# thenumbernine/lua-multigrid-poisson

Hardware: AMD Instinct MI355X
Metric: V-cycles/sec + finest-smoother achieved HBM GB/s, 3D Poisson (higher is better)
Workload: dtype f32; 1 GPU; BASELINE configs[2]: 3D Poisson 512^3 per GPU, 7-point, RB-GS 2+2, V-cycle, trilinear P, 2x2x2-average R, consistent coarse boundary, per-cycle RMS-update err; parallelism=single GPU, levels=10

## Files before the change

### lua-multigrid-poisson_amd/csrc/mgp_internal.h

```cpp
#pragma once
#include <hip/hip_runtime.h>
#include <cstdint>

namespace mgp {

constexpr int kGhost3D = 1;
constexpr int kGhostZs = 5;
constexpr int kZsHaloPre = 5, kZsHaloPost = 4, kZsHaloCoarse = 3;

struct Geo {
    int nx, ny;
    int lx, ly;
    int hw, lhw;
    int64_t nz;
    int64_t H;
    int64_t P;
    int64_t z0;
    int64_t gnz;
};

constexpr int kRealF32D = 12;

hipError_t launch_init_point_charge(int rb, int dim, void* u, void* f, Geo g, int64_t cx, int64_t cy,
                                    int64_t cz, hipStream_t s);
// ... 8 lines not shown

int half_blocks(int rb, Geo g, bool gs);
hipError_t launch_half_sweep(int rb, int dim, bool fine, int color, const void* other, const void* f, void* dst,
                             const void* old, double* partials, Geo g, double h, double cl, bool gs, hipStream_t s);
bool fresh_supported(int rb, const Geo& g);
hipError_t launch_fresh_sweep(int rb, int dim, const void* f, void* u, Geo g, double h, double cl, hipStream_t s,
                              bool store_red = true);
bool post1_supported(int rb, const Geo& g, const Geo& gc);
hipError_t launch_post_first(int rb, int dim, int linear, void* u, const void* V, const void* f, Geo g, Geo gc,
                             double h, double cl, double clc, hipStream_t s);
hipError_t launch_residual_restrict(int rb, int dim, const void* u, const void* f, void* R, Geo g, Geo gc, double h,
                                    double cl, hipStream_t s);
bool bres_supported(int rb, const Geo& g);
hipError_t launch_black_residual_restrict(int rb, int dim, void* u, const void* f, void* R, Geo g, Geo gc, double h,
                                          double cl, hipStream_t s);
hipError_t launch_rb_sweep(int rb, int dim, const void* src, const void* f, void* dst, Geo g, double h, double cl,
                           bool store_red, hipStream_t s);
hipError_t launch_residual_field_v(int rb, int dim, const void* u, const void* f, void* r, Geo g, double h, double cl,
                                   hipStream_t s);
hipError_t launch_fw_restrict(int rb, int dim, const void* r, void* R, Geo g, Geo gc, double clc, hipStream_t s);
bool resfw_supported(int rb, int dim, const Geo& g, int gz, bool dist);
hipError_t launch_resfw(int rb, int dim, const void* u, const void* f, void* R, Geo g, Geo gc, double h, double cl,
                        double clc, int gz, hipStream_t s);
hipError_t launch_prolong_correct(int rb, int dim, int linear, void* u, const void* V, Geo g, Geo gc, double clc,
                                  hipStream_t s, bool black_only = false);
hipError_t launch_sqdiff_sum(int rb, const void* a, const void* b, int64_t n, double* partials, double* out,
                             hipStream_t s, int* ctr = nullptr);
hipError_t launch_nonfinite_check(int rb, const void* p, int64_t n, int id, int* first, hipStream_t s);
hipError_t launch_metrics(int rb, const void* psi, const void* old, int64_t n, double* partials, double* out,
                          hipStream_t s);
int resnorm_blocks(int rb, Geo g);
hipError_t launch_residual_norm(int rb, int dim, const void* u, const void* f, Geo g, double h, double cl,
                                double* partials, double* out, hipStream_t s);
int sum_scratch(int n);
hipError_t launch_sum_partials(const double* partials, int n, double* out, hipStream_t s, int* ctr = nullptr);

int defect_blocks(Geo g);
int refine_add_blocks(Geo g);
int refine_partials();
hipError_t launch_defect(int dim, const double* psi64, const double* f64, float* r32, float* u32_or_null, Geo g,
                         double h, double* partials, double* out, hipStream_t s);
hipError_t launch_refine_add(double* psi64, const float* e32, Geo g, double* partials, double* out, hipStream_t s);
hipError_t launch_refine_widen(const float* src, double* dst, int64_t n, hipStream_t s);
hipError_t launch_refine_narrow(const double* src, float* dst, int64_t n, hipStream_t s);

struct FusedTuning {
    bool wide = true;
    int ys_half = -1;
    int ys_rows = 32;
    int64_t wgs = 256;
    int patch_pre = 0, patch_post = -1;
    bool fwf = true;
    int post_zc = 256;
    bool stamp_r = false;
};
FusedTuning fused_tuning_from_env();

struct LaunchInfo {
    char name[96];
    int64_t grid;
};

struct FusedArgs {
    FusedTuning tu;
    LaunchInfo* info;
    bool pre;
    int linear;
    const void* src;
    const void* f;
    void* dst;
    const void* old;
    void* R;
    const void* V;
    double* partials;
    Geo g, gc;
    double h, cl, clc;
    int zc;
    int ghost;
};
bool fused_supported(int rb, int dim, int ns, const Geo& g, const FusedTuning& tu);
hipError_t prepare_kernels(int rb);
int fused_zc(int rb, const Geo& g, bool pre, bool clz, const FusedTuning& tu);
int fused_blocks(int rb, const Geo& g, int zc, bool clz, const FusedTuning& tu);
hipError_t launch_fused(int rb, const FusedArgs& a, hipStream_t s);
bool fused_fwf_supported(int rb, int dim, bool clz, bool dist, const FusedTuning& tu);

constexpr int kBlkMaxSweeps = 2;
constexpr int kBlkTile = 8;
constexpr int kBlkTile2D = 32;
struct BlockArgs {
    bool pre;
    int linear;
    int ns;
    const void* src;
    const void* f;
    void* dst;
    void* R;
    const void* V;
    Geo g, gc;
    double h, cl, clc;
};
bool block_supported(int rb, int dim, int ns, const Geo& g);
hipError_t launch_block(int rb, int dim, const BlockArgs& a, hipStream_t s);

struct Block2Args {
    bool pre;
// ... 62 lines not shown
```

### lua-multigrid-poisson_amd/csrc/mgp_kernels.hip

```cpp
#include "mgp_device.h"

#include <cstdio>
#include <cstdlib>
#include <type_traits>
#include <utility>

namespace mgp {
namespace {




constexpr unsigned kMaxBlocks = 1u << 20;
inline unsigned nblk_gs(int64_t n)
{
    const int64_t b = (n + kBlock - 1) / kBlock;
    return (unsigned)(b < (int64_t)kMaxBlocks ? (b > 0 ? b : 1) : kMaxBlocks);
}

template <typename T>
__global__ __launch_bounds__(kBlock) void k_init(T* __restrict__ u, T* __restrict__ f, Geo g, int64_t cx, int64_t cy,
                                                 int64_t cz, int dim3)
{
    const int64_t n = g.P * g.nz;
// ... 1636 lines not shown
        const bool ox = (o == 0 && I0 + e == 0) || (o == 1 && I0 + e == cx - 1);
        auto col = [&](const T (&cc)[N + 2]) { return ox ? cc[pe] : (o ? cc[e + 2] : cc[e]); };
        const T a0 = w0 * c0[pe] + w1 * sv(col(c0), ox, false);
        const T a1 = w0 * sv(c1[pe], false, oy) + w1 * sv(col(c1), ox, oy);
        b[e] = w0 * a0 + w1 * a1;
    }
}

template <int NTL>
__device__ __forceinline__ void block_partial_t(double acc, double* partials)
{
    __shared__ double red[NTL];
    red[threadIdx.x] = acc;
    __syncthreads();
    for (int w = 512; w > 0; w >>= 1) {
        if ((int)threadIdx.x < w && (int)threadIdx.x + w < NTL) red[threadIdx.x] += red[threadIdx.x + w];
        __syncthreads();
    }
    if (threadIdx.x == 0) partials[blockIdx.x] = red[0];
}

#ifndef ZS_WPE_PRE
#define ZS_WPE_PRE 2
#endif
#ifndef ZS_PFD_PRE
#define ZS_PFD_PRE 2
#endif
#ifndef ZS_PFD_POST
#define ZS_PFD_POST 1
#endif
#ifndef ZS_PFD_PRE_CL
#define ZS_PFD_PRE_CL 1
#endif
template <typename F, int... K>
__device__ __forceinline__ void zs_unroll_impl(F& f, std::integer_sequence<int, K...>)
{
    (f(std::integral_constant<int, K>()), ...);
}
template <int U, typename F>
__device__ __forceinline__ void zs_unroll(F&& f)
{
    zs_unroll_impl(f, std::make_integer_sequence<int, U>());
}
#ifndef ZS_BQ
#define ZS_BQ 1
#endif
#ifndef ZS_RASK
#define ZS_RASK 1
#endif
constexpr bool kZsRask = ZS_RASK != 0;
#ifndef ZS_WPE_POST
#define ZS_WPE_POST 4
#endif
template <typename T, bool PRE, int LINEAR, bool ERR, bool CLZ, bool WIDE = false>
__global__ __launch_bounds__((ZsShape<T, PRE, CLZ, WIDE, PRE && LINEAR == 2>::NTL))
__attribute__((amdgpu_waves_per_eu(1, PRE ? ZS_WPE_PRE : ZS_WPE_POST))) void k_zs(const T* __restrict__ src, const T* __restrict__ f,
                                                                T* __restrict__ dst, const T* old, T* __restrict__ R,
                                                                const T* __restrict__ V, double* __restrict__ partials,
                                                                Geo g, Geo gc, Op<T, 3> op, T clc, int zc, int gz,
                                                                int patch)
{
    constexpr bool FWF = PRE && LINEAR == 2;
    using S = ZsShape<T, PRE, CLZ, WIDE, FWF>;
    constexpr int N = S::N, H = S::H, HWE = S::HWE, G = S::G, YE = S::YE, SLOT = S::SLOT, TX = S::TX,
                  TY = S::TY, NS3 = S::NS3, NTL = S::NTL;
    constexpr bool RR = PRE && LINEAR == 0;
    constexpr bool ZSRC = PRE && ERR;
    using VT = Vec<T, N>;
    using PF = ZsPrefetch<T, N>;
    constexpr int PFD = PRE ? (CLZ ? ZS_PFD_PRE : ZS_PFD_PRE_CL) : ZS_PFD_POST, NPF = PFD + 1, UNR = NPF == 3 ? 12 : 4;
    static_assert(PFD >= 1 && PFD <= 3, "prefetch distance 1..3");
    extern __shared__ __align__(16) unsigned char zs_smem[];
    T* const lds = reinterpret_cast<T*>(zs_smem);
    const int tid = threadIdx.x;

    const int tiles_x = g.nx / TX, tiles_y = g.ny / TY;
    const int b = xcd_remap(blockIdx.x, gridDim.x);
    const int tile = b % (tiles_x * tiles_y);
    const int Z0 = (b / (tiles_x * tiles_y)) * zc;
    int tx_ = tile % tiles_x, ty_ = tile / tiles_x;
    if (patch) {
        const int px = patch & 255, py = patch >> 8, per = px * py, prow = tiles_x / px;
        const int pi = tile / per, q = tile % per;
        tx_ = (pi % prow) * px + q % px;
        ty_ = (pi / prow) * py + q / px;
    }
    const int X0 = tx_ * TX, Y0 = ty_ * TY;
    const int hw = g.hw, Hh = (int)g.H;
    const int z0 = (int)g.z0, gnz = (int)g.gnz, cz0 = (int)gc.z0;
    const int64_t P = g.P;
    const int qlo = -gz, qhi = (int)g.nz - 1 + gz;

    const int wcls = S::PS ? __builtin_amdgcn_readfirstlane(tid >= S::NPAR ? 1 : 0) : 0;
    const int rt_ = S::PS ? tid - wcls * S::NPAR : tid;
    const int yr_ = S::PS ? 0 : S::yrow(tid);
    const bool on = S::PS ? rt_ < G * (wcls ? YE / 2 : S::YEV) : yr_ >= 0;
    const int gx = on ? (S::PS ? rt_ % G : S::ycol(tid)) : 0, ye = S::PS ? (on ? 2 * (rt_ / G) + wcls : wcls) : (on ? yr_ : 0);
    const int gy = Y0 - H + ye;
    const int m0 = gx * N;
    ZsCol col;
    auto lr = [&](int y) { return S::PS ? (y & 1) * S::YEV + (y >> 1) : y; };
    col.lrow = lr(ye) * HWE + m0;
    col.lym = lr(ye > 0 ? ye - 1 : ye) * HWE + m0;
    col.lyp = lr(ye < YE - 1 ? ye + 1 : ye) * HWE + m0;
    col.gm = (X0 - S::HX) / 2 + m0;
    col.x_first = gx == 0;
    col.x_last = gx == G - 1;
    col.lxm = col.x_first ? col.lrow : col.lrow - N;
    col.lxp = col.x_last ? col.lrow : col.lrow + N;
    const bool in_xy = on && gy >= 0 && gy < g.ny && col.gm >= 0 && col.gm < hw;
    col.xin = !in_xy || (col.gm > 0 && 2 * (col.gm + N) < g.nx);
    const int cgy = gy < 0 ? 0 : (gy >= g.ny ? g.ny - 1 : gy);
    const int cgm = col.gm < 0 ? 0 : (col.gm > hw - N ? hw - N : col.gm);
#if defined(ZS_HALO_ALIAS)
    const int agm = (ZS_HALO_ALIAS & 1) ? (gx < S::HXG ? cgm + S::HXG * N : (gx >= G - S::HXG ? cgm - S::HXG * N : cgm)) : cgm;
    const int agy = (ZS_HALO_ALIAS & 2) ? (ye < H ? cgy + H : (ye >= H + TY ? cgy - H : cgy)) : cgy;
    const int goff = agy * hw + agm;
#else
    const int goff = cgy * hw + cgm;
#endif
    const bool tile_xy = on && ye >= H && ye < H + TY && gx >= S::HXG && gx < G - S::HXG;
    const int ydist = ye < H ? H - ye : (ye >= H + TY ? ye - (H + TY) + 1 : 0);
    const bool need_f1 = !ZS_FHALO || PRE || ydist <= H - 1, need_f2 = !ZS_FHALO || PRE || ydist <= H - 2;
    const int zlo = Z0 - H;
    ZsDiag<T> dz;
    {
        const int nby = (gy == 0) + (gy == g.ny - 1);
        dz.db = nby == 0 ? op.dg[0] : (nby == 1 ? op.dg[1] : op.dg[2]);
        dz.yb = nby == 0 ? op.ydg[0] : (nby == 1 ? op.ydg[1] : op.ydg[2]);
        dz.de = nby == 0 ? op.dg[1] : (nby == 1 ? op.dg[2] : op.dg[3]);
        dz.ye = nby == 0 ? op.ydg[1] : (nby == 1 ? op.ydg[2] : op.ydg[3]);
        dz.left = col.gm == 0;
        dz.right = col.gm + N == hw;
    }
    const int p_end = Z0 + zc + (PRE ? (FWF ? 7 : 5) : 3);
    auto inz = [&](int q) { return z0 + q >= 0 && z0 + q < gnz; };
    auto pcl = [&](int q) { return q < qlo ? qlo : (q > qhi ? qhi : q); };
    auto slot = [&](int off, int ns, int q) {
        const int r = ns == 3 ? ((q % 3) + 3) % 3 : (q & (ns - 1));
// ... 198 lines not shown
            vstore<T, N>(slot(0, 2, p) + col.lrow, a0);
            vstore<T, N>(slot(S::OFF1, 2, p - 1) + col.lrow, o1);
            if (RO < 2) {
                vstore<T, N>(slot(S::OFF2, 2, p - 2) + col.lrow, o2);
                vstore<T, N>(slot(S::OFF3, NS3, p - 3) + col.lrow, o3);
                if (RR || FWF) vstore<T, N>(slot(S::OFF4, 2, p - 4) + col.lrow, o4);
            }
        }

        if (RO == 0) {
            const int q = p - 4;
            if (q >= Z0 && q < Z0 + zc && tile_xy) {
                if (!PRE && ERR) {
#pragma unroll
                    for (int e = 0; e < N; ++e) {
                        const double d0 = (double)W3[sl(4)].v[e] - (double)cur.o0.v[e];
                        const double d1 = (double)o4.v[e] - (double)cur.o1.v[e];
                        err = __builtin_fma(d0, d0, err);
                        err1 = __builtin_fma(d1, d1, err1);
                    }
                }
                T* dp = dst + (int64_t)q * P;
                if (!(RR || FWF) || kZsPreRed) gstore<T, N, kZsNTS>(dp + goff, W3[sl(4)]);
                gstore<T, N, kZsNTS>(dp + Hh + goff, o4);
            }
        }

        if (RR && RO == 0) {
            const int q = p - 5;
            const int pq = par(q);
            if (!kZsRask) zs_nb_load<T, N>(nr, slot(S::OFF3, NS3, q), col);
            zs_nb_load<T, N>(nk, slot(S::OFF4, 2, q), col);
            T xr[2 * N];
            {
                const T* x = xs(q - 1);
#pragma unroll
                for (int e = 0; e < 2 * N; ++e) xr[e] = x[e];
            }
            T rred[N], rblk[N], rr[2][N];
            zs_residual<T, N, CLZ, ST>(W4[sl(6)], W4[sl(5)], W4[sl(ZS_NC ? 3 : 4)], nk, W3[sl(5)], FR[sl(5)], col, pq, nbyz(q), g.nx, op,
                                   dz, rred);
            if (kZsRask)
                zs_residual_a<T, N, CLZ, ST>(AS[(RS & 1) ^ 1], W4[sl(5)], FB[sl(5)], col, 1 ^ pq, nbyz(q), g.nx, op, dz,
                                             rblk);
            else
                zs_residual<T, N, CLZ, ST>(W3[sl(6)], W3[sl(5)], W3[sl(4)], nr, W4[sl(5)], FB[sl(5)], col, 1 ^ pq, nbyz(q),
                                           g.nx, op, dz, rblk);
#pragma unroll
            for (int e = 0; e < N; ++e) {
                rr[0][e] = pq == 0 ? rred[e] : rblk[e];
                rr[1][e] = pq == 0 ? rblk[e] : rred[e];
            }
            const int dq = q - (ST ? (Z0 & ~1) : Z0);
            if (dq >= 0 && dq <= zc && tile_xy) {
                if (!even_row) {
                    if (dq < zc) {
                        T* x = xs(q);
#pragma unroll
                        for (int e = 0; e < N; ++e) {
                            x[e] = rr[0][e];
                            x[N + e] = rr[1][e];
                        }
                    }
                } else {
                    if (dq >= 1) {
#pragma unroll
                        for (int e = 0; e < N; ++e) {
                            acc[e] = acc[e] + xr[e];
                            acc[e] = acc[e] + xr[N + e];
                        }
                        if ((dq & 1) == 0) {
                            const int K = (zz0 + q - 1) >> 1, J = gy >> 1;
                            T* rowc = R + (int64_t)(K - cz0) * gc.P + (int64_t)J * gc.hw;
#pragma unroll
                            for (int e = 0; e < N; ++e) {
                                const int I = col.gm + e;
                                rowc[((I + J + K) & 1) * gc.H + (I >> 1)] = (T)0.125 * acc[e];
                            }
                        }
                    }
                    if (dq < zc) {
#pragma unroll
                        for (int e = 0; e < N; ++e) {
                            if ((dq & 1) == 0) {
                                acc[e] = rr[0][e] + rr[1][e];
                            } else {
                                acc[e] = acc[e] + rr[0][e];
                                acc[e] = acc[e] + rr[1][e];
                            }
                        }
                    }
                }
            }
        }
        if constexpr (FWF) {
            const int q = p - 5;
            const int pq = par(q);
            if (!kZsRask) zs_nb_load<T, N>(nr, slot(S::OFF3, NS3, q), col);
            zs_nb_load<T, N>(nk, slot(S::OFF4, 2, q), col);
            T rred[N], rblk[N];
            zs_residual<T, N, CLZ, ST>(W4[sl(6)], W4[sl(5)], W4[sl(ZS_NC ? 3 : 4)], nk, W3[sl(5)], FR[sl(5)], col, pq, nbyz(q), g.nx, op,
                                   dz, rred);
            if (kZsRask)
                zs_residual_a<T, N, CLZ, ST>(AS[(RS & 1) ^ 1], W4[sl(5)], FB[sl(5)], col, 1 ^ pq, nbyz(q), g.nx, op, dz,
                                             rblk);
            else
                zs_residual<T, N, CLZ, ST>(W3[sl(6)], W3[sl(5)], W3[sl(4)], nr, W4[sl(5)], FB[sl(5)], col, 1 ^ pq, nbyz(q),
                                           g.nx, op, dz, rblk);
            const bool rin = in_xy && (ST || inz(q));
            constexpr int RXH = S::RXSLOT / 2;
            const int t = ye * G + gx;
            if (ydist <= 1) {
                VT x[2];
#pragma unroll
                for (int e = 0; e < N; ++e) {
                    x[(2 * e) / N].v[(2 * e) % N] = rin ? (pq ? rblk[e] : rred[e]) : (T)0;
                    x[(2 * e + 1) / N].v[(2 * e + 1) % N] = rin ? (pq ? rred[e] : rblk[e]) : (T)0;
                }
                T* const rxw = lds + S::OFFRX + (p & 1) * S::RXSLOT + t * N;
                vstore<T, N>(rxw, x[0]);
                vstore<T, N>(rxw + RXH, x[1]);
            }
            const T wfv = (T)3 - clc, w3 = (T)3;
            const bool tile_x = gx >= S::HXG && gx < G - S::HXG;
            if (tile_x && ydist <= 1) {
                const T* rxr = lds + S::OFFRX + ((p - 1) & 1) * S::RXSLOT;
                T x[2 * N + 2];
                const VT lo = vload_lds_whole<T, N>(rxr + t * N), hi = vload_lds_whole<T, N>(rxr + RXH + t * N);
                x[0] = vload_lds_whole<T, N>(rxr + RXH + (t - 1) * N).v[N - 1];
                x[2 * N + 1] = vload_lds_whole<T, N>(rxr + (t + 1) * N).v[0];
#pragma unroll
                for (int e = 0; e < N; ++e) {
                    x[1 + e] = lo.v[e];
                    x[1 + N + e] = hi.v[e];
                }
                const int cxn = g.nx >> 1;
                VT ax;
#pragma unroll
                for (int e = 0; e < N; ++e) {
                    const int I = col.gm + e;
                    ax.v[e] = fw_axis(x[2 * e], x[2 * e + 1], x[2 * e + 2], x[2 * e + 3], I == 0 ? wfv : w3,
                                      I == cxn - 1 ? wfv : w3);
                }
                vstore<T, N>(lds + S::OFFAX + (p & 1) * S::AXSLOT + t * N, ax);
            }
            if (tid >= S::FWY * 64 && tid < S::FWY * 64 + 64) {
// ... 61 lines not shown
    for (int k = 0; k < PFD; ++k) prefetch(GEN, pb[k], zlo + k);
    int ps = zlo, pe = p_end;
    ps = ps > 6 - z0 ? ps : 6 - z0;
    ps = ps > qlo + 4 ? ps : qlo + 4;
    pe = pe < gnz - (PRE ? 1 : 2) - z0 ? pe : gnz - (PRE ? 1 : 2) - z0;
    pe = pe < qhi - PFD ? pe : qhi - PFD;
    ps += (UNR - (ps - zlo) % UNR) % UNR;
    pe -= (pe - ps + 1) % UNR;
#ifndef ZS_ALL_GENERIC
#define ZS_ALL_GENERIC 0
#endif
    if (ZS_ALL_GENERIC || pe < ps || ((z0 | Z0) & 1) || (!PRE && LINEAR == 1 && ZS_BQ && ((z0 + Z0) & 3))) ps = pe = zlo - 1;
    int p = zlo;
    const std::integral_constant<int, -1> RPL;
    const std::integral_constant<int, 0> RO0;
    auto group = [&](auto st, auto rp, auto ro, int p0, int plim) __attribute__((always_inline)) {
        zs_unroll<UNR>([&](auto kk) __attribute__((always_inline)) {
            constexpr int k = decltype(kk)::value;
            if (k == 0 || p0 + k <= plim)
                step(st, std::integral_constant<int, (k & 3)>(), rp, ro, pb[k % NPF], pb[(k + PFD) % NPF], p0 + k);
        });
    };
    for (; p < ps; p += UNR) group(GEN, RPL, RO0, p, p + UNR);
    auto steady = [&](auto rp, auto ro) __attribute__((always_inline)) {
        if constexpr (!PRE && LINEAR == 1 && ZS_BQ) {
            if (p <= pe) {
                const int K = (z0 + p) >> 1;
                bq_fill(rp, BQ[0], K);
                bq_fill(rp, BQ[1], K - 1);
            }
        }
        for (; p <= pe; p += UNR) {
#ifdef ZS_STAMP
            if (!PRE && tid == 0 && ((p - zlo) & 15) == 0 && (p - zlo) / 16 < 32) {
                const unsigned long long w = wall_clock64();
                float* out = reinterpret_cast<float*>(R) + 64 * (int)blockIdx.x + 2 * ((p - zlo) / 16);
                out[0] = __uint_as_float((unsigned)(w & 0xffffffffu));
                out[1] = __uint_as_float((unsigned)(w >> 32));
            }
#endif
            group(STY, rp, ro, p, p + UNR);
        }
    };
    if constexpr (S::PS) {
        if (((H + wcls) & 1) == 0)
            steady(std::integral_constant<int, 0>(), RO0);
        else
            steady(std::integral_constant<int, 1>(), RO0);
    } else {
        steady(RPL, RO0);
    }
    for (; p <= p_end; p += UNR) group(GEN, RPL, RO0, p, p_end);
    if constexpr (ERR && !PRE) block_partial_t<NTL>(err + err1, partials);
}

#ifndef YS_TX_F32
#define YS_TX_F32 1024
#endif
#ifndef YS_TX_F64
#define YS_TX_F64 512
#endif
template <typename T>
constexpr int ys_tx_full() { return sizeof(T) == 4 ? YS_TX_F32 : YS_TX_F64; }
template <typename T, bool PRE, int TXV = ys_tx_full<T>()>
struct YsShape {
    static constexpr int N = 16 / sizeof(T);
    static constexpr int TX = TXV;
    static constexpr int H = PRE ? 5 : 4;
    static constexpr int HX = 2 * N * ((H + 2 * N - 1) / (2 * N));
    static constexpr int HWE = TX / 2 + HX;
    static constexpr int G = HWE / N;
    static constexpr int HXG = HX / 2 / N;
    static constexpr int NTL = (G + 63) / 64 * 64;
    static constexpr int ES = 2 * G;
    static constexpr int OFF1 = 2 * ES, OFF2 = 4 * ES, OFF3 = 6 * ES, OFF4 = 10 * ES;
    static constexpr int CI = PRE ? 0 : TX / 2 + 16, CPAIRS = CI / 2, OFFC = 12 * ES;
    static constexpr size_t lds_floats = 12 * ES + 4 * CI;
    static_assert(CPAIRS <= 2 * NTL, "coarse staging: two pairs per thread");
    static_assert(NTL <= 1024, "too many threads");
    static_assert(2 * N * HXG >= H, "x halo too small");
};

#ifndef YS_PF
#define YS_PF 2
#endif
static_assert(YS_PF >= 1 && YS_PF <= 3, "prefetch distance 1..3");
template <typename T>
struct YsPrefetch {
    static constexpr int N = 16 / sizeof(T);
    Vec<T, N> u, f1, f2, o0, o1;
    Vec<T, 2> cv[2];
};

template <typename T, int N, bool CLZ, bool RES, bool AIN = false>
__device__ __forceinline__ void ys_cells(const Vec<T, N>& ym, const Vec<T, N>& cen, const Vec<T, N>& yp, T ep, T en,
                                         const Vec<T, N>& fv, const Vec<T, N>& uc, int o, int nby, int gm, int nx,
                                         bool xin, const Op<T, 2>& op, T (&out)[N], T (&ask)[N])
{
    if (!AIN) {
        ZsNb<T, N> nb;
        nb.yl = ym;
        nb.yr = yp;
        nb.ep = ep;
        nb.en = en;
        T t[N];
        zs_xsum<T, N>(cen, nb, o, t);
// ... 1670 lines not shown
    return hipSuccess;
}

template <int D>
static hipError_t pr_f32d(int linear, void* u, const void* V, Geo g, Geo gc, double clc, bool black, hipStream_t s)
{
    for (int color = black ? 1 : 0; color < 2; ++color) {
        const unsigned nb = nblk(g.H * g.nz);
        if (linear) k_prolong<float, D, 1, double><<<nb, kBlock, 0, s>>>((float*)u, (const float*)V, g, gc, clc, color);
        else k_prolong<float, D, 0, double><<<nb, kBlock, 0, s>>>((float*)u, (const float*)V, g, gc, clc, color);
        const hipError_t e = hipGetLastError();
        if (e != hipSuccess) return e;
    }
    return hipSuccess;
}

hipError_t launch_prolong_correct(int rb, int dim, int linear, void* u, const void* V, Geo g, Geo gc, double clc,
                                  hipStream_t s, bool black_only)
{
    if (rb == kRealF32D)
        return dim == 3 ? pr_f32d<3>(linear, u, V, g, gc, clc, black_only, s) : pr_f32d<2>(linear, u, V, g, gc, clc, black_only, s);
    if (rb == 8)
        return dim == 3 ? pr_t<double, 3>(linear, u, V, g, gc, clc, black_only, s)
                        : pr_t<double, 2>(linear, u, V, g, gc, clc, black_only, s);
    return dim == 3 ? pr_t<float, 3>(linear, u, V, g, gc, clc, black_only, s)
                    : pr_t<float, 2>(linear, u, V, g, gc, clc, black_only, s);
}


static int parse_patch(const char* v, int dflt)
{
    int px = 0, py = 0;
    if (!v) return dflt;
    if (std::sscanf(v, "%d,%d", &px, &py) != 2 || px < 1 || py < 1 || px > 255 || py > 255) return 0;
    return px | (py << 8);
}

FusedTuning fused_tuning_from_env()
{
    FusedTuning t;
    if (const char* v = std::getenv("MGP_ZS_WIDE")) t.wide = std::atoi(v) != 0;
    if (const char* v = std::getenv("MGP_YS_HALF")) t.ys_half = std::atoi(v);
    if (const char* v = std::getenv("MGP_YS_ROWS")) {
        const int r = std::atoi(v);
        t.ys_rows = r >= 8 && (r & 1) == 0 ? r : 32;
    }
    if (const char* v = std::getenv("MGP_ZS_WGS")) t.wgs = std::max<int64_t>(1, std::atoll(v));
    const char* vb = std::getenv("MGP_ZS_PATCH");
    const int both = parse_patch(vb, 0);
    t.patch_pre = parse_patch(std::getenv("MGP_ZS_PATCH_PRE"), both);
    t.patch_post = parse_patch(std::getenv("MGP_ZS_PATCH_POST"), vb ? both : -1);
    if (const char* v = std::getenv("MGP_ZS_FWF")) t.fwf = std::atoi(v) != 0;
    if (const char* v = std::getenv("MGP_ZS_POST_ZC")) t.post_zc = std::max(0, std::atoi(v));
    if (const char* v = std::getenv("MGP_STAMP_R")) t.stamp_r = std::atoi(v) != 0;
    return t;
}

static int zs_patch(int patch, int tiles_x, int tiles_y, unsigned nb)
{
    if (patch == -1) patch = tiles_x * tiles_y >= 4096 ? 4 | (8 << 8) : 0;
    const int px = patch & 255, py = patch >> 8;
    if (!patch || tiles_x % px || tiles_y % py || nb <= 512) return 0;
    return patch;
}

static const char* tf(bool v) { return v ? "true" : "false"; }

template <typename T, bool PRE, int LINEAR, bool ERR, bool CLZ, bool WIDE = false>
static hipError_t zs_launch(const FusedArgs& a, hipStream_t s)
{
    using S = ZsShape<T, PRE, CLZ, WIDE, PRE && LINEAR == 2>;
    const Op<T, 3> op = make_op<T, 3>(a.h, a.cl);
    const unsigned nb = (unsigned)((a.g.nx / S::TX) * (a.g.ny / S::TY) * (a.g.nz / a.zc));
    if (a.info) {
        std::snprintf(a.info->name, sizeof a.info->name, "k_zs<%s, %s, %d, %s, %s, %s>", sizeof(T) == 4 ? "float" : "double",
                      tf(PRE), LINEAR, tf(ERR), tf(CLZ), tf(WIDE));
        a.info->grid = (int64_t)nb * S::NTL;
    }
    k_zs<T, PRE, LINEAR, ERR, CLZ, WIDE><<<nb, S::NTL, S::lds_bytes, s>>>((const T*)a.src, (const T*)a.f, (T*)a.dst,
                                                                           (const T*)(a.old ? a.old : a.dst), (T*)a.R,
                                                                           (const T*)a.V, a.partials, a.g, a.gc,
                                                                           op, (T)a.clc, a.zc, a.ghost,
                                                                           zs_patch(PRE ? a.tu.patch_pre : a.tu.patch_post,
                                                                                    a.g.nx / S::TX, a.g.ny / S::TY, nb));
    return hipGetLastError();
}

#ifndef ZS_WIDE_CL
#define ZS_WIDE_CL 0
#endif
static bool zs_wide(int rb, const Geo& g, bool clz, const FusedTuning& tu)
{
    if (rb != 4 || (!clz && !ZS_WIDE_CL) || !tu.wide) return false;
    return g.nx % ZsTile<float>::TXPOST_W == 0 && g.ny % ZsTile<float>::TYPOST_W == 0;
}

static int ys_tx(int rb, const Geo& g, const FusedTuning& tu);

template <typename T, bool PRE, int LINEAR, bool ERR, bool CLZ, int TXV>
static hipError_t ys_launch_tx(const FusedArgs& a, hipStream_t s)
{
    using S = YsShape<T, PRE, TXV>;
    const Op<T, 2> op = make_op<T, 2>(a.h, a.cl);
    const unsigned nb = (unsigned)((a.g.nx / S::TX) * (a.g.ny / a.zc));
    if (a.info) {
        std::snprintf(a.info->name, sizeof a.info->name, "k_ys<%s, %s, %d, %s, %s, %d>", sizeof(T) == 4 ? "float" : "double",
                      tf(PRE), LINEAR, tf(ERR), tf(CLZ), TXV);
        a.info->grid = (int64_t)nb * S::NTL;
    }
    k_ys<T, PRE, LINEAR, ERR, CLZ, TXV><<<nb, S::NTL, 0, s>>>((const T*)a.src, (const T*)a.f, (T*)a.dst,
                                                         (const T*)(a.old ? a.old : a.dst), (T*)a.R, (const T*)a.V,
                                                         a.partials, a.g, a.gc, op, (T)a.clc, a.zc);
    return hipGetLastError();
}

template <typename T, bool PRE, int LINEAR, bool ERR, bool CLZ>
static hipError_t ys_launch(const FusedArgs& a, hipStream_t s)
{
    constexpr int F = ys_tx_full<T>();
    return ys_tx(sizeof(T), a.g, a.tu) == F ? ys_launch_tx<T, PRE, LINEAR, ERR, CLZ, F>(a, s)
                                      : ys_launch_tx<T, PRE, LINEAR, ERR, CLZ, F / 2>(a, s);
}

template <typename T, bool CLZ>
static hipError_t fused_dispatch_2d(const FusedArgs& a, hipStream_t s)
{
    const bool err = a.partials != nullptr;
    if (a.pre) return a.linear ? ys_launch<T, true, 1, false, CLZ>(a, s) : ys_launch<T, true, 0, false, CLZ>(a, s);
    if (a.linear) return err ? ys_launch<T, false, 1, true, CLZ>(a, s) : ys_launch<T, false, 1, false, CLZ>(a, s);
    return err ? ys_launch<T, false, 0, true, CLZ>(a, s) : ys_launch<T, false, 0, false, CLZ>(a, s);
}

template <typename T, bool CLZ>
static hipError_t fused_dispatch(const FusedArgs& a, hipStream_t s)
{
    const bool err = a.partials != nullptr;
#ifdef ZS_CL_AS_CLZ
    if (a.pre) return a.linear ? zs_launch<T, true, 1, false, true>(a, s) : zs_launch<T, true, 0, false, true>(a, s);
#endif
    if constexpr (std::is_same<T, float>::value && CLZ) {
        if (a.pre && a.linear == 2)
            return a.src ? zs_launch<T, true, 2, false, CLZ>(a, s) : zs_launch<T, true, 2, true, CLZ>(a, s);
    }
    if (a.pre && a.linear == 2) return hipErrorInvalidValue;
    if (a.pre && !a.src)
        return a.linear ? zs_launch<T, true, 1, true, CLZ>(a, s) : zs_launch<T, true, 0, true, CLZ>(a, s);
    if (a.pre) return a.linear ? zs_launch<T, true, 1, false, CLZ>(a, s) : zs_launch<T, true, 0, false, CLZ>(a, s);
    if constexpr (std::is_same<T, float>::value && CLZ) {
        if (zs_wide(4, a.g, true, a.tu)) {
            if (a.linear)
                return err ? zs_launch<T, false, 1, true, CLZ, true>(a, s) : zs_launch<T, false, 1, false, CLZ, true>(a, s);
            return err ? zs_launch<T, false, 0, true, CLZ, true>(a, s) : zs_launch<T, false, 0, false, CLZ, true>(a, s);
        }
    }
    if constexpr (std::is_same<T, float>::value && !CLZ && ZS_WIDE_CL) {
        if (!err && zs_wide(4, a.g, false, a.tu))
            return a.linear ? zs_launch<T, false, 1, false, CLZ, true>(a, s) : zs_launch<T, false, 0, false, CLZ, true>(a, s);
    }
    if (a.linear) return err ? zs_launch<T, false, 1, true, CLZ>(a, s) : zs_launch<T, false, 1, false, CLZ>(a, s);
    return err ? zs_launch<T, false, 0, true, CLZ>(a, s) : zs_launch<T, false, 0, false, CLZ>(a, s);
}

static void zs_tile(int rb, int& tx, int& ty, int pre = -1, bool clz = true, bool wide = false)
{
    const int xa = rb == 4 ? ZsTile<float>::TXPRE : ZsTile<double>::TXPRE;
    const int xc = rb == 4 ? ZsTile<float>::TXPRE_CL : ZsTile<double>::TXPRE_CL;
    const int xb = rb == 4 ? ZsTile<float>::TXPOST : ZsTile<double>::TXPOST;
    const int a = rb == 4 ? ZsTile<float>::TYPRE : ZsTile<double>::TYPRE;
    const int ac = rb == 4 ? ZsTile<float>::TYPRE_CL : ZsTile<double>::TYPRE_CL;
    const int b = rb == 4 ? ZsTile<float>::TYPOST : ZsTile<double>::TYPOST;
    const int xp = clz ? xa : xc, yp = clz ? a : ac;
    auto mx = [](int u, int v, int w) { return u > v ? (u > w ? u : w) : (v > w ? v : w); };
    tx = pre < 0 ? mx(xa, xb, xc) : (pre ? xp : xb);
    ty = pre < 0 ? mx(a, b, ac) : (pre ? yp : b);
    if (pre == 0 && wide) {
        tx = ZsTile<float>::TXPOST_W;
        ty = ZsTile<float>::TYPOST_W;
    }
}

static int ys_rows(const Geo& g, const FusedTuning& tu)
{
    int r = tu.ys_rows;
    while (r > 8 && g.ny % r != 0) r /= 2;
    return r;
}

static int ys_tx(int rb, const Geo& g, const FusedTuning& tu)
{
    const int mode = tu.ys_half;
    const int64_t target = tu.wgs;
    const int full = rb == 4 ? ys_tx_full<float>() : ys_tx_full<double>();
    if (mode == 0 || g.nx % (full / 2) != 0) return full;
    if (mode == 1 || g.nx % full != 0) return full / 2;
    return (int64_t)(g.nx / full) * (g.ny / ys_rows(g, tu)) < target ? full / 2 : full;
}

// ... 11 lines not shown
{
    if (g.gnz == 1 && g.nz == 1) return ys_rows(g, tu);
    int TX, TY;
    zs_tile(rb, TX, TY, pre ? 1 : 0, clz, !pre && zs_wide(rb, g, clz, tu));
    const int64_t target = tu.wgs;
    const int64_t tiles = (int64_t)(g.nx / TX) * (g.ny / TY);
    int64_t chunks = 1;
    while (tiles * chunks < target && g.nz / (chunks * 2) >= 16) chunks *= 2;
    while (!pre && tu.post_zc > 0 && g.nz / chunks > tu.post_zc && g.nz / (chunks * 2) >= 16) chunks *= 2;
    return (int)(g.nz / chunks);
}

int fused_blocks(int rb, const Geo& g, int zc, bool clz, const FusedTuning& tu)
{
    if (g.gnz == 1 && g.nz == 1) return (g.nx / ys_tx(rb, g, tu)) * (g.ny / zc);
    int TX, TY;
    zs_tile(rb, TX, TY, 0, clz, zs_wide(rb, g, clz, tu));
    return (int)((int64_t)(g.nx / TX) * (g.ny / TY) * (g.nz / zc));
}

int fused_halo(bool pre) { return pre ? 5 : 4; }

bool fused_fwf_supported(int rb, int dim, bool clz, bool dist, const FusedTuning& tu)
{
    return rb == 4 && dim == 3 && clz && !dist && tu.fwf;
}

template <typename T, bool CLZ>
static hipError_t fused_attr()
{
    const int pre = (int)ZsShape<T, true, CLZ>::lds_bytes, post = (int)ZsShape<T, false, CLZ>::lds_bytes;
    const auto A = hipFuncAttributeMaxDynamicSharedMemorySize;
    if constexpr (std::is_same<T, float>::value && CLZ) {
        const int w = (int)ZsShape<T, true, CLZ, false, true>::lds_bytes;
        hipError_t e = hipFuncSetAttribute((const void*)k_zs<T, true, 2, false, CLZ>, A, w);
        if (e == hipSuccess) e = hipFuncSetAttribute((const void*)k_zs<T, true, 2, true, CLZ>, A, w);
        if (e != hipSuccess) return e;
    }
    if constexpr (std::is_same<T, float>::value && CLZ) {
        const int w = (int)ZsShape<T, false, CLZ, true>::lds_bytes;
        hipError_t e = hipFuncSetAttribute((const void*)k_zs<T, false, 0, false, CLZ, true>, A, w);
        if (e == hipSuccess) e = hipFuncSetAttribute((const void*)k_zs<T, false, 0, true, CLZ, true>, A, w);
        if (e == hipSuccess) e = hipFuncSetAttribute((const void*)k_zs<T, false, 1, false, CLZ, true>, A, w);
        if (e == hipSuccess) e = hipFuncSetAttribute((const void*)k_zs<T, false, 1, true, CLZ, true>, A, w);
        if (e != hipSuccess) return e;
    }
    if constexpr (std::is_same<T, float>::value && !CLZ && ZS_WIDE_CL) {
        const int w = (int)ZsShape<T, false, CLZ, true>::lds_bytes;
        hipError_t e = hipFuncSetAttribute((const void*)k_zs<T, false, 0, false, CLZ, true>, A, w);
        if (e == hipSuccess) e = hipFuncSetAttribute((const void*)k_zs<T, false, 1, false, CLZ, true>, A, w);
        if (e != hipSuccess) return e;
    }
    hipError_t e = hipFuncSetAttribute((const void*)k_zs<T, true, 0, false, CLZ>, A, pre);
    if (e == hipSuccess) e = hipFuncSetAttribute((const void*)k_zs<T, true, 1, false, CLZ>, A, pre);
    if (e == hipSuccess) e = hipFuncSetAttribute((const void*)k_zs<T, true, 0, true, CLZ>, A, pre);
    if (e == hipSuccess) e = hipFuncSetAttribute((const void*)k_zs<T, true, 1, true, CLZ>, A, pre);
    if (e == hipSuccess) e = hipFuncSetAttribute((const void*)k_zs<T, false, 0, false, CLZ>, A, post);
    if (e == hipSuccess) e = hipFuncSetAttribute((const void*)k_zs<T, false, 0, true, CLZ>, A, post);
    if (e == hipSuccess) e = hipFuncSetAttribute((const void*)k_zs<T, false, 1, false, CLZ>, A, post);
    if (e == hipSuccess) e = hipFuncSetAttribute((const void*)k_zs<T, false, 1, true, CLZ>, A, post);
    return e;
}

#ifdef TAIL_PROF
constexpr int kTailStaticLds = 1024;
#else
constexpr int kTailStaticLds = 0;
#endif
template <typename T>
static hipError_t tail_c_attr();

template <typename T, int D>
static hipError_t tail_attr()
{
    hipError_t e = hipFuncSetAttribute((const void*)k_tail<T, D, 0>, hipFuncAttributeMaxDynamicSharedMemorySize,
                                       (int)kTailMaxLds - kTailStaticLds);
    if (e == hipSuccess)
        e = hipFuncSetAttribute((const void*)k_tail<T, D, 1>, hipFuncAttributeMaxDynamicSharedMemorySize,
                                (int)kTailMaxLds - kTailStaticLds);
    return e;
}

template <typename T>
static hipError_t blk_attr();

hipError_t prepare_kernels(int rb)
{
    hipError_t e = hipSuccess;
#define MGP_CHAIN(x) \
    if (e == hipSuccess) e = (x)
    if (rb == 4) {
        MGP_CHAIN((fused_attr<float, true>()));
        MGP_CHAIN((fused_attr<float, false>()));
        MGP_CHAIN((tail_attr<float, 2>()));
        MGP_CHAIN((tail_attr<float, 3>()));
        MGP_CHAIN((tail_c_attr<float>()));
        MGP_CHAIN((blk_attr<float>()));
        MGP_CHAIN((blk2_attr(4)));
    } else {
        MGP_CHAIN((fused_attr<double, true>()));
        MGP_CHAIN((fused_attr<double, false>()));
        MGP_CHAIN((tail_attr<double, 2>()));
        MGP_CHAIN((tail_attr<double, 3>()));
        MGP_CHAIN((tail_c_attr<double>()));
        MGP_CHAIN((blk_attr<double>()));
        MGP_CHAIN((blk2_attr(8)));
// ... 410 lines not shown
```

Baseline: 997.0 V-cycles/s (512^3-cell slabs, whole job).

## Split fused pre-smooth+restrict kernel into producer/consumer wave groups

Adds k_zs_split, a warp-specialized variant of the fused pre-smoothing z-streaming kernel. One wave group runs the first three relax stages and prefetches, while another runs the fourth relax, the residual and the 2x2x2 restriction from LDS, with forcing rows staged through new LDS slots. It is enabled by default for float, CLZ, pre-smooth, non-linear cases and can be disabled with MGP_ZS_SPLIT. The aim is to overlap global loads with the later stages and cut per-thread register pressure. The cost is more waves per block, more LDS and extra barriers per step.

After: 1036 V-cycles/s (512^3-cell slabs, whole job), median of 6. +3.9%, better.

```diff
diff --git a/lua-multigrid-poisson_amd/csrc/mgp_internal.h b/lua-multigrid-poisson_amd/csrc/mgp_internal.h
--- a/lua-multigrid-poisson_amd/csrc/mgp_internal.h
+++ b/lua-multigrid-poisson_amd/csrc/mgp_internal.h
@@ -84,6 +84,7 @@
     int patch_pre = 0, patch_post = -1;
     bool fwf = true;
     int post_zc = 256;
+    bool split = true;
     bool stamp_r = false;
 };
 FusedTuning fused_tuning_from_env();
diff --git a/lua-multigrid-poisson_amd/csrc/mgp_kernels.hip b/lua-multigrid-poisson_amd/csrc/mgp_kernels.hip
--- a/lua-multigrid-poisson_amd/csrc/mgp_kernels.hip
+++ b/lua-multigrid-poisson_amd/csrc/mgp_kernels.hip
@@ -1712,6 +1712,61 @@
 #ifndef ZS_WPE_POST
 #define ZS_WPE_POST 4
 #endif
+__device__ __forceinline__ void zs_tile_xy(int tile, int tiles_x, int patch, int& tx, int& ty)
+{
+    tx = tile % tiles_x;
+    ty = tile / tiles_x;
+    if (patch) {
+        const int px = patch & 255, py = patch >> 8, per = px * py, prow = tiles_x / px;
+        const int pi = tile / per, q = tile % per;
+        tx = (pi % prow) * px + q % px;
+        ty = (pi / prow) * py + q / px;
+    }
+}
+
+template <typename T, int N>
+__device__ __forceinline__ void zs_restrict_avg(const T (&rr)[2][N], const T (&xr)[2 * N], T (&acc)[N], int dq, int zc,
+                                                bool even_row, T* xw, T* __restrict__ R, int K, int J, int gm, int cz0,
+                                                const Geo& gc)
+{
+    if (!even_row) {
+        if (dq < zc) {
+#pragma unroll
+            for (int e = 0; e < N; ++e) {
+                xw[e] = rr[0][e];
+                xw[N + e] = rr[1][e];
+            }
+        }
+    } else {
+        if (dq >= 1) {
+#pragma unroll
+            for (int e = 0; e < N; ++e) {
+                acc[e] = acc[e] + xr[e];
+                acc[e] = acc[e] + xr[N + e];
+            }
+            if ((dq & 1) == 0) {
+                T* rowc = R + (int64_t)(K - cz0) * gc.P + (int64_t)J * gc.hw;
+#pragma unroll
+                for (int e = 0; e < N; ++e) {
+                    const int I = gm + e;
+                    rowc[((I + J + K) & 1) * gc.H + (I >> 1)] = (T)0.125 * acc[e];
+                }
+            }
+        }
+        if (dq < zc) {
+#pragma unroll
+            for (int e = 0; e < N; ++e) {
+                if ((dq & 1) == 0) {
+                    acc[e] = rr[0][e] + rr[1][e];
+                } else {
+                    acc[e] = acc[e] + rr[0][e];
+                    acc[e] = acc[e] + rr[1][e];
+                }
+            }
+        }
+    }
+}
+
 template <typename T, bool PRE, int LINEAR, bool ERR, bool CLZ, bool WIDE = false>
 __global__ __launch_bounds__((ZsShape<T, PRE, CLZ, WIDE, PRE && LINEAR == 2>::NTL))
 __attribute__((amdgpu_waves_per_eu(1, PRE ? ZS_WPE_PRE : ZS_WPE_POST))) void k_zs(const T* __restrict__ src, const T* __restrict__ f,
@@ -1738,13 +1793,8 @@
     const int b = xcd_remap(blockIdx.x, gridDim.x);
     const int tile = b % (tiles_x * tiles_y);
     const int Z0 = (b / (tiles_x * tiles_y)) * zc;
-    int tx_ = tile % tiles_x, ty_ = tile / tiles_x;
-    if (patch) {
-        const int px = patch & 255, py = patch >> 8, per = px * py, prow = tiles_x / px;
-        const int pi = tile / per, q = tile % per;
-        tx_ = (pi % prow) * px + q % px;
-        ty_ = (pi / prow) * py + q / px;
-    }
+    int tx_, ty_;
+    zs_tile_xy(tile, tiles_x, patch, tx_, ty_);
     const int X0 = tx_ * TX, Y0 = ty_ * TY;
     const int hw = g.hw, Hh = (int)g.H;
     const int z0 = (int)g.z0, gnz = (int)g.gnz, cz0 = (int)gc.z0;
@@ -2049,46 +2099,8 @@
                 rr[1][e] = pq == 0 ? rblk[e] : rred[e];
             }
             const int dq = q - (ST ? (Z0 & ~1) : Z0);
-            if (dq >= 0 && dq <= zc && tile_xy) {
-                if (!even_row) {
-                    if (dq < zc) {
-                        T* x = xs(q);
-#pragma unroll
-                        for (int e = 0; e < N; ++e) {
-                            x[e] = rr[0][e];
-                            x[N + e] = rr[1][e];
-                        }
-                    }
-                } else {
-                    if (dq >= 1) {
-#pragma unroll
-                        for (int e = 0; e < N; ++e) {
-                            acc[e] = acc[e] + xr[e];
-                            acc[e] = acc[e] + xr[N + e];
-                        }
-                        if ((dq & 1) == 0) {
-                            const int K = (zz0 + q - 1) >> 1, J = gy >> 1;
-                            T* rowc = R + (int64_t)(K - cz0) * gc.P + (int64_t)J * gc.hw;
-#pragma unroll
-                            for (int e = 0; e < N; ++e) {
-                                const int I = col.gm + e;
-                                rowc[((I + J + K) & 1) * gc.H + (I >> 1)] = (T)0.125 * acc[e];
-                            }
-                        }
-                    }
-                    if (dq < zc) {
-#pragma unroll
-                        for (int e = 0; e < N; ++e) {
-                            if ((dq & 1) == 0) {
-                                acc[e] = rr[0][e] + rr[1][e];
-                            } else {
-                                acc[e] = acc[e] + rr[0][e];
-                                acc[e] = acc[e] + rr[1][e];
-                            }
-                        }
-                    }
-                }
-            }
+            if (dq >= 0 && dq <= zc && tile_xy)
+                zs_restrict_avg<T, N>(rr, xr, acc, dq, zc, even_row, xs(q), R, (zz0 + q - 1) >> 1, gy >> 1, col.gm, cz0, gc);
         }
         if constexpr (FWF) {
             const int q = p - 5;
@@ -2256,6 +2268,277 @@
     }
     for (; p <= p_end; p += UNR) group(GEN, RPL, RO0, p, p_end);
     if constexpr (ERR && !PRE) block_partial_t<NTL>(err + err1, partials);
+}
+
+template <typename T>
+struct ZsSplit {
+    using S = ZsShape<T, true, true>;
+    static_assert(S::XPAIR && S::H == 5 && S::NS3 == 4 && kZsRask, "the split follows k_zs's 64 x 32 PRE layout");
+    static constexpr int NTW = S::TC / 64;
+    static constexpr int NW = 2 * NTW + 4, NTL = 64 * NW, WMIX = NW - 1;
+    static constexpr int MA = S::YT2 - S::YT2S, MB = 2 * S::G;
+    static_assert(NTW == 4 && S::NTL == 64 * 7 && S::YT2S == 64 * 6 && S::YT0 == 64 * 5 && MA + MB <= 64, "wave order");
+    static constexpr int wave_kind(int w) { return w == WMIX ? 2 : (w < 2 * NTW ? w >= NTW : ((w - 2 * NTW) & 1)); }
+    static constexpr int local_wave(int w) { return w < 2 * NTW ? w % NTW : NTW + (w - 2 * NTW) / 2; }
+    static constexpr int BT1 = S::YT0 + MB;
+    static __device__ __forceinline__ int b_yrow(int t)
+    {
+        if (t < S::YT0) return S::yrow(t);
+        if (t < BT1) return t - S::YT0 < S::G ? S::H - 1 : S::H + S::TY;
+        return -1;
+    }
+    static __device__ __forceinline__ int b_ycol(int t) { return t < S::YT0 ? S::ycol(t) : (t - S::YT0) % S::G; }
+    static constexpr int FROWS = S::TY + 2, FSLOT = FROWS * S::HWE;
+    static constexpr int OFFFR = (int)(S::lds_bytes / sizeof(T)), OFFFB = OFFFR + 4 * FSLOT;
+    static constexpr size_t lds_bytes = (size_t)(OFFFB + 4 * FSLOT) * sizeof(T);
+    static_assert(NTL <= 1024 && NW <= 12, "too many waves for 168 VGPRs");
+    static_assert(lds_bytes <= 160 * 1024, "LDS");
+};
+
+template <typename T, bool ZSRC>
+__global__ __launch_bounds__((ZsSplit<T>::NTL)) void k_zs_split(const T* __restrict__ src, const T* __restrict__ f,
+                                                                 T* __restrict__ dst, T* __restrict__ R, Geo g, Geo gc,
+                                                                 Op<T, 3> op, int zc, int gz, int patch)
+{
+    using SP = ZsSplit<T>;
+    using S = typename SP::S;
+    constexpr int N = S::N, H = S::H, HWE = S::HWE, G = S::G, YE = S::YE, SLOT = S::SLOT, TX = S::TX, TY = S::TY,
+                  NS3 = S::NS3;
+    using VT = Vec<T, N>;
+    using PF = ZsPrefetch<T, N>;
+    constexpr int PFD = ZS_PFD_PRE, NPF = PFD + 1, UNR = NPF == 3 ? 12 : 4;
+    static_assert(PFD >= 1 && PFD <= 3, "prefetch distance 1..3");
+    extern __shared__ __align__(16) unsigned char zs_smem[];
+    T* const lds = reinterpret_cast<T*>(zs_smem);
+    const int tid = threadIdx.x;
+
+    const int tiles_x = g.nx / TX, tiles_y = g.ny / TY;
+    const int b = xcd_remap(blockIdx.x, gridDim.x);
+    const int tile = b % (tiles_x * tiles_y);
+    const int Z0 = (b / (tiles_x * tiles_y)) * zc;
+    int tx_, ty_;
+    zs_tile_xy(tile, tiles_x, patch, tx_, ty_);
+    const int X0 = tx_ * TX, Y0 = ty_ * TY;
+    const int hw = g.hw, Hh = (int)g.H;
+    const int z0 = (int)g.z0, gnz = (int)g.gnz, cz0 = (int)gc.z0;
+    const int64_t P = g.P;
+    const int qlo = -gz, qhi = (int)g.nz - 1 + gz;
+
+    const int wv = __builtin_amdgcn_readfirstlane(tid >> 6), lane = tid & 63;
+    const int wk = SP::wave_kind(wv), lw = SP::local_wave(wv);
+    const bool grp_b = wk == 1 || (wk == 2 && lane >= SP::MA);
+    const int lt = wk == 2 ? (grp_b ? S::YT0 + lane - SP::MA : S::YT2S + lane) : 64 * lw + lane;
+    const int yr_ = grp_b ? SP::b_yrow(lt) : S::yrow(lt);
+    const bool on = yr_ >= 0;
+    const int gx = on ? (grp_b ? SP::b_ycol(lt) : S::ycol(lt)) : 0, ye = on ? yr_ : 0;
+    const int gy = Y0 - H + ye;
+    const int m0 = gx * N;
+    ZsCol col;
+    col.lrow = ye * HWE + m0;
+    col.lym = (ye > 0 ? ye - 1 : ye) * HWE + m0;
+    col.lyp = (ye < YE - 1 ? ye + 1 : ye) * HWE + m0;
+    col.gm = (X0 - S::HX) / 2 + m0;
+    col.x_first = gx == 0;
+    col.x_last = gx == G - 1;
+    col.lxm = col.x_first ? col.lrow : col.lrow - N;
+    col.lxp = col.x_last ? col.lrow : col.lrow + N;
+    const bool in_xy = on && gy >= 0 && gy < g.ny && col.gm >= 0 && col.gm < hw;
+    col.xin = true;
+    const int cgy = gy < 0 ? 0 : (gy >= g.ny ? g.ny - 1 : gy);
+    const int cgm = col.gm < 0 ? 0 : (col.gm > hw - N ? hw - N : col.gm);
+    const int goff = cgy * hw + cgm;
+    const bool tile_xy = on && ye >= H && ye < H + TY && gx >= S::HXG && gx < G - S::HXG;
+    const bool frow = on && ye >= H - 1 && ye <= H + TY;
+    const int lf = frow ? (ye - (H - 1)) * HWE + m0 : 0;
+    auto fslot = [&](int off, int q) { return lds + off + (q & 3) * SP::FSLOT + lf; };
+    const int zlo = Z0 - H;
+    const ZsDiag<T> dz = {};
+    const int p_end = Z0 + zc + 6;
+    auto inz = [&](int q) { return z0 + q >= 0 && z0 + q < gnz; };
+    auto pcl = [&](int q) { return q < qlo ? qlo : (q > qhi ? qhi : q); };
+    auto slot = [&](int off, int ns, int q) { return lds + off + (q & (ns - 1)) * SLOT; };
+    const int rowpar = (gy + z0) & 1;
+    auto par = [&](int q) { return rowpar ^ (q & 1); };
+    const VT vz = vzero<T, N>();
+
+    for (int i = tid; i < (int)(SP::lds_bytes / sizeof(T)); i += SP::NTL) lds[i] = (T)0;
+    __syncthreads();
+
+    int ps = zlo, pe = p_end;
+    ps = ps > 7 - z0 ? ps : 7 - z0;
+    ps = ps > qlo + 4 ? ps : qlo + 4;
+    pe = pe < gnz - 1 - z0 ? pe : gnz - 1 - z0;
+    pe = pe < qhi - PFD ? pe : qhi - PFD;
+    ps += (UNR - (ps - zlo) % UNR) % UNR;
+    pe -= (pe - ps + 1) % UNR;
+    if (pe < ps || ((z0 | Z0) & 1)) ps = pe = zlo - 1;
+    const std::false_type GEN;
+    const std::true_type STY;
+    auto run = [&](auto&& prefetch, auto&& step) __attribute__((always_inline)) {
+        PF pb[NPF];
+#pragma unroll
+        for (int k = 0; k < PFD; ++k) prefetch(GEN, pb[k], zlo + k);
+        int p = zlo;
+        auto group = [&](auto st, int p0, int plim) __attribute__((always_inline)) {
+            zs_unroll<UNR>([&](auto kk) __attribute__((always_inline)) {
+                constexpr int k = decltype(kk)::value;
+                if (k == 0 || p0 + k <= plim) {
+                    step(st, std::integral_constant<int, (k & 3)>(), pb[k % NPF], pb[(k + PFD) % NPF], p0 + k);
+                    lds_barrier();
+                }
+            });
+        };
+        for (; p < ps; p += UNR) group(GEN, p, p + UNR);
+        for (; p <= pe; p += UNR) group(STY, p, p + UNR);
+        for (; p <= p_end; p += UNR) group(GEN, p, p_end);
+    };
+
+    const T* const src_black = ZSRC ? nullptr : src + Hh;
+    auto prefetch_a = [&](auto st, PF& r, int p) __attribute__((always_inline)) {
+        constexpr bool ST = decltype(st)::value;
+        if (ST) {
+            const int64_t pP = (int64_t)p * P;
+            if constexpr (ZSRC)
+                r.u = vzero<T, N>();
+            else
+                r.u = gload<T, N, kZsNTL>(src_black + pP + goff);
+            r.f1 = gload<T, N, kZsNTL>(f + (pP - P) + goff);
+            r.f2 = gload<T, N, kZsNTL>(f + (pP - 2 * P) + Hh + goff);
+        } else {
+            if constexpr (ZSRC)
+                r.u = vzero<T, N>();
+            else
+                r.u = gload<T, N, kZsNTL>(src_black + (int64_t)pcl(p) * P + goff);
+            r.f1 = gload<T, N, kZsNTL>(f + (int64_t)pcl(p - 1) * P + goff);
+            r.f2 = gload<T, N, kZsNTL>(f + (int64_t)pcl(p - 2) * P + Hh + goff);
+        }
+    };
+    VT W0[4], W1[4], W2[4], FR[4];
+#pragma unroll
+    for (int i = 0; i < 4; ++i) W0[i] = W1[i] = W2[i] = FR[i] = vz;
+    auto step_a = [&](auto st, auto rt, const PF& cur, PF& nxt, int p, int ro) __attribute__((always_inline)) {
+        constexpr bool ST = decltype(st)::value;
+        constexpr int RS = decltype(rt)::value;
+        auto sl = [](int k) constexpr { return (RS - k) & 3; };
+        if (ST) p = (p & ~1) | ((H + RS) & 1);
+        zs_hold<T, N>(cur.u);
+        zs_hold<T, N>(cur.f1);
+        zs_hold<T, N>(cur.f2);
+        asm volatile("" ::: "memory");
+        if (ST || p + PFD <= p_end) prefetch_a(st, nxt, p + PFD);
+        ZsNb<T, N> n1, n2, n3;
+        VT a0 = cur.u;
+        if (!ST && !inz(p)) a0 = vz;
+        W0[sl(0)] = a0;
+        zs_nb_load<T, N>(n1, slot(0, 2, p - 1), col);
+        VT o1 = zs_relax<T, N, true, ST>(W0[sl(2)], W0[sl(1)], W0[sl(0)], n1, cur.f1, col, par(p - 1), 0, g.nx, op, dz);
+        if (!ST && !inz(p - 1)) o1 = vz;
+        W1[sl(1)] = o1;
+        VT o2 = vz, o3 = vz;
+        if (ro < 2) {
+            zs_nb_load<T, N>(n2, slot(S::OFF1, 2, p - 2), col);
+            o2 = zs_relax<T, N, true, ST>(W1[sl(3)], W1[sl(2)], W1[sl(1)], n2, cur.f2, col, 1 ^ par(p - 2), 0, g.nx, op, dz);
+            if (!ST && !inz(p - 2)) o2 = vz;
+            W2[sl(2)] = o2;
+            zs_nb_load<T, N>(n3, slot(S::OFF2, 2, p - 3), col);
+            o3 = zs_relax<T, N, true, ST>(W2[sl(4)], W2[sl(3)], W2[sl(2)], n3, FR[sl(3)], col, par(p - 3), 0, g.nx, op, dz);
+            if (!ST && !inz(p - 3)) o3 = vz;
+        }
+        if (in_xy) {
+            vstore<T, N>(slot(0, 2, p) + col.lrow, a0);
+            vstore<T, N>(slot(S::OFF1, 2, p - 1) + col.lrow, o1);
+            if (ro < 2) {
+                vstore<T, N>(slot(S::OFF2, 2, p - 2) + col.lrow, o2);
+                vstore<T, N>(slot(S::OFF3, NS3, p - 3) + col.lrow, o3);
+            }
+            if (frow) {
+                vstore<T, N>(fslot(SP::OFFFR, p - 3), FR[sl(3)]);
+                vstore<T, N>(fslot(SP::OFFFB, p - 2), cur.f2);
+            }
+        }
+        FR[sl(1)] = cur.f1;
+    };
+
+    auto prefetch_b = [](auto, PF&, int) {};
+    VT W3[4], W4[4], FB[4];
+    T AS[2][N], acc[N];
+#pragma unroll
+    for (int e = 0; e < N; ++e) AS[0][e] = AS[1][e] = acc[e] = (T)0;
+#pragma unroll
+    for (int i = 0; i < 4; ++i) W3[i] = W4[i] = FB[i] = vz;
+    const bool even_row = (gy & 1) == 0;
+    T* const xbase = lds + S::OFFX + (((ye + (H & 1)) >> 1) * G + gx) * 2 * N;
+    auto xs = [&](int q) { return xbase + (q & 1) * (S::XPAIRS * G * 2 * N); };
+    auto step_b = [&](auto st, auto rt, auto tw, int p) __attribute__((always_inline)) {
+        constexpr bool ST = decltype(st)::value;
+        constexpr int RS = decltype(rt)::value;
+        auto sl = [](int k) constexpr { return (RS - k) & 3; };
+        if (ST) p = (p & ~1) | ((H + RS) & 1);
+        const int zz0 = ST ? (z0 & ~1) : z0;
+        ZsNb<T, N> n4, nk;
+        const VT fb = vload<T, N>(fslot(SP::OFFFB, p - 5));
+        W3[sl(4)] = vload<T, N>(slot(S::OFF3, NS3, p - 4) + col.lrow);
+        zs_nb_load<T, N>(n4, slot(S::OFF3, NS3, p - 5), col);
+        VT o4 = zs_relax_a<T, N, true, ST>(W3[sl(6)], W3[sl(5)], W3[sl(4)], n4, fb, col, 1 ^ par(p - 5), 0, g.nx, op, dz,
+                                           AS[RS & 1]);
+        if (!ST && !inz(p - 5)) o4 = vz;
+        W4[sl(5)] = o4;
+        if (in_xy) vstore<T, N>(slot(S::OFF4, 2, p - 5) + col.lrow, o4);
+        if constexpr (decltype(tw)::value) {
+            {
+                const int q = p - 5;
+                if (q >= Z0 && q < Z0 + zc && tile_xy) gstore<T, N, kZsNTS>(dst + (int64_t)q * P + Hh + goff, o4);
+            }
+            const int q = p - 6;
+            const int pq = par(q);
+            zs_nb_load<T, N>(nk, slot(S::OFF4, 2, q), col);
+            T xr[2 * N];
+            {
+                const T* x = xs(q - 1);
+#pragma unroll
+                for (int e = 0; e < 2 * N; ++e) xr[e] = x[e];
+            }
+            T rred[N], rblk[N], rr[2][N];
+            const VT fr = vload<T, N>(fslot(SP::OFFFR, q));
+            zs_residual<T, N, true, ST>(W4[sl(7)], W4[sl(6)], W4[sl(5)], nk, W3[sl(6)], fr, col, pq, 0, g.nx, op, dz, rred);
+            zs_residual_a<T, N, true, ST>(AS[(RS & 1) ^ 1], W4[sl(6)], FB[sl(6)], col, 1 ^ pq, 0, g.nx, op, dz, rblk);
+#pragma unroll
+            for (int e = 0; e < N; ++e) {
+                rr[0][e] = pq == 0 ? rred[e] : rblk[e];
+                rr[1][e] = pq == 0 ? rblk[e] : rred[e];
+            }
+            const int dq = q - (ST ? (Z0 & ~1) : Z0);
+            if (dq >= 0 && dq <= zc && tile_xy)
+                zs_restrict_avg<T, N>(rr, xr, acc, dq, zc, even_row, xs(q), R, (zz0 + q - 1) >> 1, gy >> 1, col.gm, cz0, gc);
+            FB[sl(5)] = fb;
+        }
+    };
+
+    if (wk == 0) {
+        const int wrole = S::wave_role(lw);
+        run(prefetch_a, [&](auto st, auto rt, const PF& cur, PF& nxt, int p) __attribute__((always_inline)) {
+            step_a(st, rt, cur, nxt, p, decltype(st)::value ? wrole : 0);
+        });
+    } else if (wk == 1) {
+        if (lw < SP::NTW)
+            run(prefetch_b, [&](auto st, auto rt, const PF& cur, PF& nxt, int p) __attribute__((always_inline)) {
+                step_b(st, rt, STY, p);
+            });
+        else
+            run(prefetch_b, [&](auto st, auto rt, const PF& cur, PF& nxt, int p) __attribute__((always_inline)) {
+                step_b(st, rt, GEN, p);
+            });
+    } else {
+        run(
+            [&](auto st, PF& r, int p) __attribute__((always_inline)) {
+                if (!grp_b) prefetch_a(st, r, p);
+            },
+            [&](auto st, auto rt, const PF& cur, PF& nxt, int p) __attribute__((always_inline)) {
+                if (!grp_b) step_a(st, rt, cur, nxt, p, 2);
+                asm volatile("" ::: "memory");
+                if (grp_b) step_b(st, rt, GEN, p);
+            });
+    }
 }
 
 #ifndef YS_TX_F32
@@ -4032,6 +4315,7 @@
     t.patch_post = parse_patch(std::getenv("MGP_ZS_PATCH_POST"), vb ? both : -1);
     if (const char* v = std::getenv("MGP_ZS_FWF")) t.fwf = std::atoi(v) != 0;
     if (const char* v = std::getenv("MGP_ZS_POST_ZC")) t.post_zc = std::max(0, std::atoi(v));
+    if (const char* v = std::getenv("MGP_ZS_SPLIT")) t.split = std::atoi(v) != 0;
     if (const char* v = std::getenv("MGP_STAMP_R")) t.stamp_r = std::atoi(v) != 0;
     return t;
 }
@@ -4066,6 +4350,23 @@
     return hipGetLastError();
 }
 
+template <bool ZSRC>
+static hipError_t zs_split_launch(const FusedArgs& a, hipStream_t s)
+{
+    using SP = ZsSplit<float>;
+    using S = SP::S;
+    const Op<float, 3> op = make_op<float, 3>(a.h, a.cl);
+    const unsigned nb = (unsigned)((a.g.nx / S::TX) * (a.g.ny / S::TY) * (a.g.nz / a.zc));
+    if (a.info) {
+        std::snprintf(a.info->name, sizeof a.info->name, "k_zs_split<float, %s>", tf(ZSRC));
+        a.info->grid = (int64_t)nb * SP::NTL;
+    }
+    k_zs_split<float, ZSRC><<<nb, SP::NTL, SP::lds_bytes, s>>>((const float*)a.src, (const float*)a.f, (float*)a.dst,
+                                                                (float*)a.R, a.g, a.gc, op, a.zc, a.ghost,
+                                                                zs_patch(a.tu.patch_pre, a.g.nx / S::TX, a.g.ny / S::TY, nb));
+    return hipGetLastError();
+}
+
 #ifndef ZS_WIDE_CL
 #define ZS_WIDE_CL 0
 #endif
@@ -4123,6 +4424,9 @@
             return a.src ? zs_launch<T, true, 2, false, CLZ>(a, s) : zs_launch<T, true, 2, true, CLZ>(a, s);
     }
     if (a.pre && a.linear == 2) return hipErrorInvalidValue;
+    if constexpr (std::is_same<T, float>::value && CLZ) {
+        if (a.pre && !a.linear && a.tu.split) return a.src ? zs_split_launch<false>(a, s) : zs_split_launch<true>(a, s);
+    }
     if (a.pre && !a.src)
         return a.linear ? zs_launch<T, true, 1, true, CLZ>(a, s) : zs_launch<T, true, 0, true, CLZ>(a, s);
     if (a.pre) return a.linear ? zs_launch<T, true, 1, false, CLZ>(a, s) : zs_launch<T, true, 0, false, CLZ>(a, s);
@@ -4240,6 +4544,11 @@
         if (e != hipSuccess) return e;
     }
     hipError_t e = hipFuncSetAttribute((const void*)k_zs<T, true, 0, false, CLZ>, A, pre);
+    if constexpr (std::is_same<T, float>::value && CLZ) {
+        const int w = (int)ZsSplit<float>::lds_bytes;
+        if (e == hipSuccess) e = hipFuncSetAttribute((const void*)k_zs_split<float, false>, A, w);
+        if (e == hipSuccess) e = hipFuncSetAttribute((const void*)k_zs_split<float, true>, A, w);
+    }
     if (e == hipSuccess) e = hipFuncSetAttribute((const void*)k_zs<T, true, 1, false, CLZ>, A, pre);
     if (e == hipSuccess) e = hipFuncSetAttribute((const void*)k_zs<T, true, 0, true, CLZ>, A, pre);
     if (e == hipSuccess) e = hipFuncSetAttribute((const void*)k_zs<T, true, 1, true, CLZ>, A, pre);
```
